# vincentjzy/OpenCorr

Hardware: AMD Instinct MI355X
Metric: converged POIs/sec (FFTCC+ICGN2D1, 33x33 subset) (higher is better)
Workload: dtype f32

## Files before the change

opencorr_amd/csrc/capi.hip:

```cpp
#include "capi_internal.h"

namespace ochip_capi {

thread_local std::string g_last_error;

int fail(int code, const char* fmt, ...) {
    char buf[512];
    va_list ap;
    va_start(ap, fmt);
    vsnprintf(buf, sizeof(buf), fmt, ap);
    va_end(ap);
    g_last_error = buf;
    return code;
}

static std::once_flag g_rocfft_once;
void rocfft_init_once() {
    std::call_once(g_rocfft_once, [] { rocfft_setup(); });
}

int create_engine(int kind, int rx, int ry, int rz, float conv, float stop, int device, oc_hip_engine** out) {
    if (!out) return fail(OC_HIP_ERR_INVALID, "null output handle");
    *out = nullptr;
    if (rx < 1 || ry < 1 || ((kind == OC_HIP_FFTCC3D || kind == OC_HIP_ICGN3D1) && rz < 1))
// ... 152 lines not shown

int run_icgn2d(oc_hip_engine* e, float* d_pois, int stride_f, size_t count, const float* d_offsets) {
    if (!e->img || e->img->ndim != 2) return fail(OC_HIP_ERR_INVALID, "ICGN2D: set_images2d has not been called");
    if (!e->ref_ready || !e->tar_ready)
        return fail(OC_HIP_ERR_INVALID, "ICGN2D: prepare() has not been called since the last set_images");
    const ImagePair& im = *e->img;
    OC_TRY(check_image2d_limits("ICGN2D", im, 1ull << 28));
    const int dof = (e->kind == OC_HIP_ICGN2D1 || e->kind == OC_HIP_ICLM2D1) ? 6 : 12;
    const bool lm = e->is_iclm();
    const bool onepass = e->arith_onepass && !lm;
    if (onepass && d_offsets)
        return fail(OC_HIP_ERR_UNSUPPORTED, "ICGN2D%d: centre offsets are not supported under arith_onepass = 1 (the one-pass kernel keeps "
                                            "integer local coordinates in a per-workgroup table); set arith_onepass = 0 for this call", dof == 6 ? 1 : 2);
    if (onepass && e->self_adaptive)
        return fail(OC_HIP_ERR_UNSUPPORTED, "ICGN2D%d: self-adaptive subset radii are not supported under arith_onepass = 1 (the one-pass "
                                            "kernel runs one radius per launch); set arith_onepass = 0", dof == 6 ? 1 : 2);
    int rx = e->rx, ry = e->ry;
    if (e->self_adaptive) {
        OC_TRY(e->cursors.reserve(2 * sizeof(int)));
        OC_HIP_TRY(ochip::launch_poi2d_max_radius(d_pois, stride_f, count, e->cursors.as<int>(), e->stream));
        int mx[2] = {0, 0};
        OC_HIP_TRY(hipMemcpyAsync(mx, e->cursors.p, sizeof(mx), hipMemcpyDeviceToHost, e->stream));
        OC_HIP_TRY(hipStreamSynchronize(e->stream));
        rx = mx[0] > 0 ? mx[0] : 1;
        ry = mx[1] > 0 ? mx[1] : 1;
        if (rx > 4096 || ry > 4096) return fail(OC_HIP_ERR_UNSUPPORTED, "ICGN2D: self-adaptive subset radius %d x %d is not plausible", rx, ry);
    }
    ochip::Icgn2dParams P = {im.ref_ptr(), e->gx.as<float>(), e->gy.as<float>(), e->coef.as<float>(),
                             im.dy,        im.dx,              rx,                ry,
                             e->conv,      e->stop,            d_offsets,         nullptr,
                             e->self_adaptive ? 1 : 0,
                             lm ? std::log((double)e->lm_lambda) : 0.0,
                             e->lm_alpha,  e->lm_beta,         e->arith_fma,      nullptr};
    const long long N = (2LL * rx + 1) * (2LL * ry + 1);
    int variant = e->icgn2d_variant;
    if (variant < 0) {
        const long long passes = ((2LL * rx + 1) * (2LL * ry + 1) + 63) / 64;
        variant = dof == 12 ? (passes <= 28 && count >= 32768 ? 4 : 3) : (passes <= 19 && count >= 32768 ? 5 : 2);
    }
    if (e->self_adaptive && (e->icgn2d_variant < 0 || ochip::icgn2d_variant_uses_table(variant))) {
        const long long passes_sa = (N + 63) / 64;
        const bool crowded = 3 * (2 * 4 * passes_sa * 256) > (160 * 1024 - 2048);
        variant = crowded ? 7 : (dof == 12 ? 3 : 2);
    }
    if (lm) variant = 1;
#if OC_BUILD_AB
    const bool band = variant == 9 && !lm && !e->self_adaptive && ochip::icgn2d_band_supported(dof, rx, ry);
#else
    const bool band = false;
#endif
    if (variant == 9 && !band) variant = dof == 12 ? 3 : 2;
    if (onepass && N > ochip::icgn2d_onepass_max_samples())
        return fail(OC_HIP_ERR_UNSUPPORTED, "ICGN2D%d: subset %dx%d (%lld samples) exceeds the one-pass kernel's on-chip limit of %d samples",
                    dof == 6 ? 1 : 2, 2 * rx + 1, 2 * ry + 1, N, ochip::icgn2d_onepass_max_samples());
    if (onepass) variant = dof == 6 ? 5 : 4;
    if (!band && !onepass && N > ochip::icgn2d_max_samples(variant)) variant = 1;
    if (!band && !onepass && N > ochip::icgn2d_max_samples(variant))
        return fail(OC_HIP_ERR_UNSUPPORTED, "ICGN2D%d: subset %dx%d (%lld samples) exceeds the on-chip limit of %d samples",
                    dof == 6 ? 1 : 2, 2 * rx + 1, 2 * ry + 1, N, ochip::icgn2d_max_samples(variant));
    if (variant == 8 && !lm) {
        OC_TRY(e->setup_recs.reserve(count * (size_t)ochip::icgn2d_setup_record_floats(dof) * sizeof(float)));
        P.setup = e->setup_recs.as<float>();
    }
    const size_t kMaxGrid = 1u << 30;
    e->setup_cache_last = 0;
    const bool cached = e->icgn2d_setup_cache && !onepass && !lm && !band && !d_offsets && !e->self_adaptive && (variant == 4 || variant == 5) &&
// ... 472 lines not shown
    for (oc_hip_engine* r : e->replicas) {
        oc_hip_engine* twin = nullptr;
        for (oc_hip_engine* d : donor->replicas)
            if (d->device == r->device && d->img && d->img->ndim == donor->img->ndim && d->img->dx == donor->img->dx &&
                d->img->dy == donor->img->dy && d->img->dz == donor->img->dz)
                twin = d;
        if (twin && r->device != e->device) {
            std::lock_guard<std::mutex> rlock(r->mu);
            r->img = twin->img;
            r->ref_ready = r->tar_ready = false;
            r->ref_generation++;
        } else {
            OC_TRY(replicate_images(e, r));
        }
    }
    return OC_HIP_OK;
}

static int clone_engine(const oc_hip_engine* e, int device, oc_hip_engine** out) {
    OC_TRY(create_engine(e->kind, e->rx, e->ry, e->rz, e->conv, e->stop, device, out));
    oc_hip_engine* r = *out;
    r->is_replica = true;
    r->lm_lambda = e->lm_lambda;
    r->lm_alpha = e->lm_alpha;
    r->lm_beta = e->lm_beta;
    r->icgn2d_tile_px = e->icgn2d_tile_px;
    r->icgn2d_variant = e->icgn2d_variant;
    r->self_adaptive = e->self_adaptive;
    r->icgn2d_xcd = e->icgn2d_xcd;
    r->arith_fma = e->arith_fma;
    r->arith_onepass = e->arith_onepass;
    r->icgn2d_split_chunks = e->icgn2d_split_chunks;
    r->icgn2d_setup_cache = e->icgn2d_setup_cache;
    r->fftcc2d_fused = e->fftcc2d_fused;
    r->fftcc3d_fused = e->fftcc3d_fused;
    r->fftcc3d_planes_blocks = e->fftcc3d_planes_blocks;
    r->icgn3d_mapping = e->icgn3d_mapping;
    r->icgn3d_tile_vox = e->icgn3d_tile_vox;
    r->fftcc3d_tile_vox = e->fftcc3d_tile_vox;
    r->host_chunk = e->host_chunk;
    r->group_allgather = e->group_allgather;
    r->group_force_rccl = e->group_force_rccl;
    return OC_HIP_OK;
}

static int rehome(oc_hip_engine* e, int device) {
    int ndev = 0;
    OC_HIP_TRY(hipGetDeviceCount(&ndev));
    if (device < 0 || device >= ndev) return fail(OC_HIP_ERR_INVALID, "device %d out of range [0,%d)", device, ndev);
    OC_HIP_TRY(hipSetDevice(e->device));
    drain_engine(e);
    e->tail_marked = false;
    clear_events(e);
    e->fft.destroy();
    e->fft.work_fwd.release();
    e->fft.work_inv.release();
    for (DevBuf* b : {&e->gx, &e->gy, &e->gz, &e->coef, &e->coef_gx, &e->coef_gy, &e->tmp, &e->poi_stage, &e->off_stage, &e->cursors,
                      &e->perm, &e->tiles, &e->perm_slots, &e->split_scratch, &e->split_tmp, &e->prefilter_tmp, &e->st_box, &e->st_counts, &e->st_start, &e->st_cursor, &e->st_slots,
                      &e->st_order, &e->st_recs, &e->st_fallback, &e->win, &e->freq, &e->norms, &e->flags, &e->group_mirror,
                      &e->group_off_mirror, &e->setup_cache_recs, &e->setup_cache_xy, &e->setup_cache_word})
        b->release();
    e->setup_cache_valid = false;
    e->setup_cache_last = 0;
    e->img.reset();
    e->ref_ready = e->tar_ready = false;
    e->st_count = 0;
    if (e->order_ev) { (void)hipEventDestroy(e->order_ev); e->order_ev = nullptr; }
    if (e->switch_ev) { (void)hipEventDestroy(e->switch_ev); e->switch_ev = nullptr; }
    if (e->group_ev) { (void)hipEventDestroy(e->group_ev); e->group_ev = nullptr; }
    for (hipEvent_t ev : e->chunk_done) (void)hipEventDestroy(ev);
    for (hipEvent_t ev : e->chunk_in) (void)hipEventDestroy(ev);
    e->chunk_done.clear();
    e->chunk_in.clear();
    if (e->copy_stream) { (void)hipStreamDestroy(e->copy_stream); e->copy_stream = nullptr; }
    if (e->copy_in_stream) { (void)hipStreamDestroy(e->copy_in_stream); e->copy_in_stream = nullptr; }
    for (hipEvent_t ev : e->split_ev) (void)hipEventDestroy(ev);
    e->split_ev.clear();
    if (e->aux_stream) { (void)hipStreamSynchronize(e->aux_stream); (void)hipStreamDestroy(e->aux_stream); e->aux_stream = nullptr; }
    (void)hipStreamDestroy(e->own_stream);
    e->own_stream = nullptr;
    OC_HIP_TRY(hipSetDevice(device));
    e->device = device;
    OC_HIP_TRY(hipStreamCreateWithFlags(&e->own_stream, hipStreamNonBlocking));
    e->stream = e->own_stream;
    return OC_HIP_OK;
}

int oc_hip_set_devices(oc_hip_engine* e, const int* device_ids, int n_devices) {
    OC_TRY(check_engine(e));
    DeviceScope device_scope;
    if (e->is_replica) return fail(OC_HIP_ERR_INVALID, "set_devices: this handle is a group member");
    if (!device_ids || n_devices < 1) return fail(OC_HIP_ERR_INVALID, "set_devices: need at least one device id");
    if (e->kind == OC_HIP_CALIBRATION || e->kind == OC_HIP_STEREOVISION)
        return fail(OC_HIP_ERR_UNSUPPORTED, "set_devices: Calibration / Stereovision handles stay on the device they were created for");
    if (n_devices > 1 && (e->kind == OC_HIP_STRAIN || e->kind == OC_HIP_REGION_FIT))
        return fail(OC_HIP_ERR_UNSUPPORTED, "set_devices: Strain / RegionFit need every neighbour of a POI and stay on one device");
    int ndev = 0;
    OC_HIP_TRY(hipGetDeviceCount(&ndev));
// ... 141 lines not shown

int oc_hip_set_tuning(oc_hip_engine* e, const char* key, int value) {
    OC_TRY(check_engine(e));
    if (!key) return fail(OC_HIP_ERR_INVALID, "null tuning key");
    std::lock_guard<std::mutex> lock(e->mu);
    const std::string k(key);
    if (k == "icgn2d_variant") {
        if (value < -1 || value >= ochip::icgn2d_variant_count())
            return fail(OC_HIP_ERR_INVALID, "icgn2d_variant %d out of range [-1 (automatic), %d)", value, ochip::icgn2d_variant_count());
        if (value >= 0 && !ochip::icgn2d_variant_built(value))
            return fail(OC_HIP_ERR_UNSUPPORTED, "icgn2d_variant %d is an A/B partner that only the A/B build of the library contains "
                                               "(python -m opencorr_amd.build --ab)", value);
        e->icgn2d_variant = value;
    } else if (k == "icgn2d_xcd" || k == "xcd") {
        e->icgn2d_xcd = value != 0;
    } else if (k == "arith_fma") {
        if (value != 0 && !(e->is_icgn2d() || e->kind == OC_HIP_ICGN3D1))
            return fail(OC_HIP_ERR_UNSUPPORTED, "arith_fma: only the ICGN2D1 / ICGN2D2 / ICLM2D1 / ICLM2D2 / ICGN3D1 engines have a fused-arithmetic build");
        e->arith_fma = value != 0;
    } else if (k == "arith_onepass") {
        if (value != 0 && !(e->kind == OC_HIP_ICGN2D1 || e->kind == OC_HIP_ICGN2D2))
            return fail(OC_HIP_ERR_UNSUPPORTED, "arith_onepass: only the ICGN2D1 / ICGN2D2 engines have a one-pass build");
        e->arith_onepass = value != 0;
    } else if (k == "icgn2d_split_chunks") {
#if !OC_BUILD_AB
        if (value != 0)
            return fail(OC_HIP_ERR_UNSUPPORTED, "icgn2d_split_chunks belongs to icgn2d_variant 8, an A/B partner that only the A/B build of the "
                                                "library contains (python -m opencorr_amd.build --ab)");
#endif
        if (value < 0 || value > 256) return fail(OC_HIP_ERR_INVALID, "icgn2d_split_chunks must be 0 (back to back) ... 256");
        e->icgn2d_split_chunks = value;
    } else if (k == "icgn2d_setup_cache") {
        e->icgn2d_setup_cache = value != 0;
    } else if (k == "icgn2d_tile_px") {
        if (value < 0 || (value > 0 && value < 16)) return fail(OC_HIP_ERR_INVALID, "icgn2d_tile_px must be 0 (off) or >= 16");
        e->icgn2d_tile_px = value;
    } else if (k == "fftcc2d_fused") {
        e->fftcc2d_fused = value == 2 ? 2 : (value != 0);
    } else if (k == "fftcc3d_fused") {
#if !OC_BUILD_AB
        if (value == 2)
            return fail(OC_HIP_ERR_UNSUPPORTED, "fftcc3d_fused = 2 (the 32^3 kernel of rounds 1 - 5) is an A/B partner that only the A/B build of the "
                                                "library contains (python -m opencorr_amd.build --ab)");
#endif
        e->fftcc3d_fused = value == 2 ? 2 : (value != 0);
    } else if (k == "fftcc3d_tile_vox") {
        if (value < 0 || (value > 0 && value < 8)) return fail(OC_HIP_ERR_INVALID, "fftcc3d_tile_vox must be 0 (off) or >= 8");
        e->fftcc3d_tile_vox = value;
    } else if (k == "icgn3d_tile_vox") {
        if (value < 0 || (value > 0 && value < 8)) return fail(OC_HIP_ERR_INVALID, "icgn3d_tile_vox must be 0 (off) or >= 8");
        e->icgn3d_tile_vox = value;
    } else if (k == "icgn3d_mapping") {
#if !OC_BUILD_AB
        if (value != 0)
            return fail(OC_HIP_ERR_UNSUPPORTED, "icgn3d_mapping = 1 (the row mapping, measured 12 - 25 %% slower) is an A/B partner that only "
                                               "the A/B build of the library contains (python -m opencorr_amd.build --ab)");
#endif
        e->icgn3d_mapping = value != 0;
    } else if (k == "fftcc3d_planes_blocks") {
        if (value < 0 || value > 4096) return fail(OC_HIP_ERR_INVALID, "fftcc3d_planes_blocks must be 0 (default) ... 4096");
        e->fftcc3d_planes_blocks = value;
    } else if (k == "single_combine") {
        e->single_combine = value != 0;
    } else if (k == "host_chunk") {
        if (value < 0 || (value > 0 && value < 16384)) return fail(OC_HIP_ERR_INVALID, "host_chunk must be 0 (off) or >= 16384 POIs");
        e->host_chunk = value;
// ... 21 lines not shown
        e->ref_ready = true;
        for (oc_hip_engine* r : e->replicas) OC_TRY(oc_hip_prepare_ref(r));
        return OC_HIP_OK;
    }
    if (im.ndim == 2) {
        OC_TRY(e->gx.reserve(bytes));
        OC_TRY(e->gy.reserve(bytes));
        OC_HIP_TRY(ochip::launch_grad2d(im.ref_ptr(), im.dy, im.dx, e->gx.as<float>(), e->gy.as<float>(), e->stream));
    } else {
        OC_TRY(e->gx.reserve(bytes));
        OC_TRY(e->gy.reserve(bytes));
        OC_TRY(e->gz.reserve(bytes));
        OC_HIP_TRY(ochip::launch_grad3d(im.ref_ptr(), im.dz, im.dy, im.dx, e->gx.as<float>(), e->gy.as<float>(),
                                        e->gz.as<float>(), e->stream));
    }
    e->ref_ready = true;
    e->ref_generation++;
    OC_TRY(mark_tail(e));
    for (oc_hip_engine* r : e->replicas) OC_TRY(oc_hip_prepare_ref(r));
    OC_HIP_TRY(hipSetDevice(e->device));
    return OC_HIP_OK;
}

int oc_hip_prepare_tar(oc_hip_engine* e) {
    OC_ACTIVATE(e);
    if (!e->is_icgn()) return OC_HIP_OK;
    if (!e->img) return fail(OC_HIP_ERR_INVALID, "prepare: set_images has not been called");
    std::lock_guard<std::mutex> lock(e->mu);
    TailGuard tail(e);
    OC_TRY(order_after_default_stream(e));
    const ImagePair& im = *e->img;
    if (im.ndim == 2) {
        OC_TRY(check_image2d_limits(e->kind == OC_HIP_NR2D1 ? "NR2D1" : "ICGN2D", im, e->kind == OC_HIP_NR2D1 ? 1ull << 26 : 1ull << 28));
        OC_TRY(e->coef.reserve(im.count() * 16 * sizeof(float)));
        OC_HIP_TRY(ochip::launch_bspline2d_lut(im.tar_ptr(), im.dy, im.dx, e->coef.as<float>(), e->stream));
        if (e->kind == OC_HIP_NR2D1) {
            OC_TRY(e->gx.reserve(im.count() * sizeof(float)));
            OC_TRY(e->gy.reserve(im.count() * sizeof(float)));
            OC_TRY(e->coef_gx.reserve(im.count() * 16 * sizeof(float)));
            OC_TRY(e->coef_gy.reserve(im.count() * 16 * sizeof(float)));
            OC_HIP_TRY(ochip::launch_grad2d(im.tar_ptr(), im.dy, im.dx, e->gx.as<float>(), e->gy.as<float>(), e->stream));
            OC_HIP_TRY(ochip::launch_bspline2d_lut(e->gx.as<float>(), im.dy, im.dx, e->coef_gx.as<float>(), e->stream));
            OC_HIP_TRY(ochip::launch_bspline2d_lut(e->gy.as<float>(), im.dy, im.dx, e->coef_gy.as<float>(), e->stream));
        }
    } else {
        OC_TRY(e->coef.reserve(im.count() * sizeof(float)));
        OC_TRY(e->prefilter_tmp.reserve(im.count() * sizeof(float)));
        OC_HIP_TRY(ochip::launch_bspline3d_prefilter(im.tar_ptr(), im.dz, im.dy, im.dx, e->coef.as<float>(),
                                                     e->prefilter_tmp.as<float>(), e->stream));
    }
    e->tar_ready = true;
    OC_TRY(mark_tail(e));
    for (oc_hip_engine* r : e->replicas) OC_TRY(oc_hip_prepare_tar(r));
    OC_HIP_TRY(hipSetDevice(e->device));
    return OC_HIP_OK;
}

int oc_hip_prepare(oc_hip_engine* e) {
    OC_TRY(oc_hip_prepare_ref(e));
    return oc_hip_prepare_tar(e);
}

}


extern "C" {

static int compute_impl(oc_hip_engine* e, void* pois, const float* offsets, size_t count, size_t stride_bytes, int memory) {
// ... 276 lines not shown
    std::lock_guard<std::mutex> lock(e->mu);
    e->self_adaptive = enable != 0;
    for (oc_hip_engine* r : e->replicas) OC_TRY(oc_hip_set_self_adaptive(r, enable));
    return OC_HIP_OK;
}

int oc_hip_synchronize(oc_hip_engine* e) {
    OC_ACTIVATE(e);
    OC_HIP_TRY(hipStreamSynchronize(e->stream));
    return OC_HIP_OK;
}

int oc_hip_get_kind(const oc_hip_engine* e, int* kind) {
    OC_TRY(check_engine(e));
    if (!kind) return fail(OC_HIP_ERR_INVALID, "null kind");
    *kind = e->kind;
    return OC_HIP_OK;
}

int oc_hip_get_field(const oc_hip_engine* e, const char* name, const float** ptr, size_t* count) {
    OC_TRY(check_engine(e));
    if (!name || !ptr || !count) return fail(OC_HIP_ERR_INVALID, "null argument");
    *ptr = nullptr;
    *count = 0;
    if (!e->img) return fail(OC_HIP_ERR_INVALID, "get_field(%s): no images set", name);
    const size_t n = e->img->count();
    const std::string s(name);
    if (s == "ref") { *ptr = e->img->ref_ptr(); *count = n; }
    else if (s == "tar") { *ptr = e->img->tar_ptr(); *count = n; }
    else if (s == "gx" && e->ref_ready) { *ptr = e->gx.as<float>(); *count = n; }
    else if (s == "gy" && e->ref_ready) { *ptr = e->gy.as<float>(); *count = n; }
    else if (s == "gz" && e->ref_ready && e->is3d()) { *ptr = e->gz.as<float>(); *count = n; }
    else if (s == "lut" && e->tar_ready && !e->is3d()) { *ptr = e->coef.as<float>(); *count = n * 16; }
    else if (s == "lut_gx" && e->tar_ready && e->kind == OC_HIP_NR2D1) { *ptr = e->coef_gx.as<float>(); *count = n * 16; }
    else if (s == "lut_gy" && e->tar_ready && e->kind == OC_HIP_NR2D1) { *ptr = e->coef_gy.as<float>(); *count = n * 16; }
    else if (s == "coef" && e->tar_ready && e->is3d()) { *ptr = e->coef.as<float>(); *count = n; }
    else return fail(OC_HIP_ERR_INVALID, "get_field: '%s' is unknown or not built yet", name);
    return OC_HIP_OK;
}

int oc_hip_read_field(oc_hip_engine* e, const char* name, float* host_dst, size_t count) {
    OC_ACTIVATE(e);
    const float* p = nullptr;
    size_t n = 0;
    OC_TRY(oc_hip_get_field(e, name, &p, &n));
    if (!host_dst || count != n) return fail(OC_HIP_ERR_INVALID, "read_field(%s): expected %zu floats, got %zu", name, n, count);
    OC_HIP_TRY(hipMemcpyAsync(host_dst, p, n * sizeof(float), hipMemcpyDeviceToHost, e->stream));
    OC_HIP_TRY(hipStreamSynchronize(e->stream));
    return OC_HIP_OK;
}

int oc_hip_profile_enable(oc_hip_engine* e, int enable) {
    OC_TRY(check_engine(e));
    std::lock_guard<std::mutex> lock(e->mu);
    e->prof = enable != 0;
    return OC_HIP_OK;
}

int oc_hip_profile_reset(oc_hip_engine* e) {
    OC_ACTIVATE(e);
    std::lock_guard<std::mutex> lock(e->mu);
    OC_HIP_TRY(hipStreamSynchronize(e->stream));
    clear_events(e);
    return OC_HIP_OK;
}

// ... 32 lines not shown
```

opencorr_amd/csrc/capi_internal.h:

```cpp
#pragma once
#include "../../include/opencorr_hip.h"

#include <hip/hip_runtime.h>
#include <rocfft/rocfft.h>

#include <dlfcn.h>

#include <algorithm>
#include <atomic>
#include <chrono>
#include <cmath>
#include <condition_variable>
#include <cstdarg>
#include <cstdio>
#include <cstdlib>
#include <cstring>
#include <memory>
#include <mutex>
#include <string>
#include <thread>
#include <vector>

#if __has_include(<rccl/rccl.h>)
#include <rccl/rccl.h>
// ... 129 lines not shown
    int rx = 0, ry = 0, rz = 0;
    float conv = 0.001f, stop = 10.f;
    hipStream_t own_stream = nullptr;
    hipStream_t stream = nullptr;
    hipEvent_t order_ev = nullptr;
    hipEvent_t switch_ev = nullptr;
    bool tail_marked = false;
    std::shared_ptr<ImagePair> img;
    DevBuf gx, gy, gz, coef;
    DevBuf coef_gx, coef_gy;
    DevBuf tmp;
    DevBuf prefilter_tmp;
    bool ref_ready = false, tar_ready = false;
    DevBuf poi_stage, off_stage;
    DevBuf cursors;
    DevBuf perm, tiles, perm_slots;
    DevBuf setup_recs;
    DevBuf setup_cache_recs, setup_cache_xy, setup_cache_word;
    struct SetupCacheKey {
        size_t count = 0;
        int stride_f = 0, variant = -1, dof = 0, rx = 0, ry = 0, arith_fma = 0, height = 0, width = 0;
        const void *ref = nullptr, *gx = nullptr, *gy = nullptr;
        unsigned long long ref_generation = 0;
        bool operator==(const SetupCacheKey& o) const {
            return count == o.count && stride_f == o.stride_f && variant == o.variant && dof == o.dof && rx == o.rx && ry == o.ry &&
                   arith_fma == o.arith_fma && height == o.height && width == o.width && ref == o.ref && gx == o.gx && gy == o.gy &&
                   ref_generation == o.ref_generation;
        }
    } setup_cache_key;
    bool setup_cache_valid = false;
    unsigned long long ref_generation = 0;
    unsigned setup_cache_epoch = 0;
    int setup_cache_last = 0;
    int icgn2d_setup_cache = 1;
    DevBuf split_scratch, split_tmp;
    float st_radius = 0.f, st_zncc = 0.9f;
    int st_nmin = 0, st_approx = 1, st_ndim = 0;
    size_t st_count = 0;
    ochip::StrainGrid st_grid{};
    DevBuf st_box, st_counts, st_start, st_cursor, st_slots, st_order, st_recs, st_fallback;
    float cal_i[13] = {}, cal_e[6] = {};
    float cal_K[9] = {}, cal_R[9] = {}, cal_T[3] = {}, cal_P[12] = {};
    float cal_conv = 0.001f;
    int cal_iter = 40, cal_h = 0, cal_w = 0;
    DevBuf cal_map_x, cal_map_y, cal_stage;
    oc_hip_engine* stereo_cam[2] = {nullptr, nullptr};
    float stereo_F[9] = {};
    float lm_lambda = 100.f, lm_alpha = 0.1f, lm_beta = 10.f;
    int icgn2d_tile_px = 128;
    FftPlans fft;
    DevBuf win, freq, norms, flags;
    int icgn2d_variant = -1;
    bool self_adaptive = false;
    int icgn2d_xcd = 1;
    int arith_fma = 0;
    int arith_onepass = 0;
    int fftcc2d_fused = 1;
    int fftcc3d_fused = 1;
    int fftcc3d_planes_blocks = 0;
    int fftcc3d_tile_vox = 64;
    int icgn3d_tile_vox = 64;
    int icgn3d_mapping = 0;
    hipStream_t copy_stream = nullptr, copy_in_stream = nullptr;
    hipStream_t aux_stream = nullptr;
    std::vector<hipEvent_t> split_ev;
    int icgn2d_split_chunks = 0;
// ... 159 lines not shown
```

opencorr_amd/csrc/icgn2d.hip:

```cpp
#include <atomic>
#include <cstdlib>
#include <type_traits>

#include "dic2d_device.h"
#include "oc_kernels.h"
#ifndef OC_ABLATE2D
#define OC_ABLATE2D 0
#endif
#ifndef OC_SWEEP_BARRIER
#define OC_SWEEP_BARRIER -1
#endif
#ifndef OC_SWEEP_PRIO
#define OC_SWEEP_PRIO 0
#endif
#ifndef OC_SETUP_BATCH
#define OC_SETUP_BATCH 6
#endif
#ifndef OC_HESS_BATCH
#define OC_HESS_BATCH 6
#endif
#ifndef OC_NUM_BATCH
#define OC_NUM_BATCH 6
#endif
#ifndef OC_V5_G
// ... 116 lines not shown
    int rx = P.rx, ry = P.ry;
    if (P.self_adaptive) {
        rx = (int)wave_bcast(rec, poi2d::SRX);
        ry = (int)wave_bcast(rec, poi2d::SRY);
        if (rx < 0 || ry < 0 || (2 * rx + 1) * (2 * ry + 1) > NTA * kWave) {
            if (lane == 0) poi[poi2d::ZNCC] = zncc_in >= 0 ? -3.f : zncc_in;
            leave();
            return;
        }
    }
    float offx = 0.f, offy = 0.f;
    if constexpr (OFFS) {
        offx = uni(P.offsets[2 * idx]);
        offy = uni(P.offsets[2 * idx + 1]);
    }

    const bool guard_geo = py - ry < 0 || px - rx < 0 || py + ry > height - 1 || px + rx > width - 1;
    const bool guard_data = fabsf(u_in) >= width || fabsf(v_in) >= height || zncc_in < 0 || isnan(u_in) || isnan(v_in);
    if (guard_geo || (guard_data && !cache_fill)) {
        if (lane == 0) poi[poi2d::ZNCC] = zncc_in >= 0 ? -3.f : zncc_in;
        leave();
        return;
    }
    const int W = 2 * rx + 1, N = W * (2 * ry + 1);
    const float fN = (float)N;
    const int NT = (N + kWave - 1) / kWave;
    const int NF = N / kWave;
    const int q64 = kWave / W, r64 = kWave - q64 * W;
    const int r0 = lane / W;
    const int c0 = lane - r0 * W;
    const unsigned goff = (unsigned)__builtin_amdgcn_readfirstlane((((int)py - ry) * width + ((int)px - rx)) * 4);
    const __amdgpu_buffer_rsrc_t r_gx = make_rsrc(P.gx), r_gy = make_rsrc(P.gy), r_ref = make_rsrc(P.ref);
    const LutPlanes4 r_lut(P.lut, height, width);
    const unsigned w4 = (unsigned)width * 4u;
    auto soff = [&](const SampleWalk& w) { return __umul24((unsigned)w.r, w4) + ((unsigned)w.c << 2); };

    auto tab_at = [&](int t) { return tab_xy[t * kWave + lane]; };
    auto off_at = [&](int t) { return tab_off[t * kWave + lane]; };

    float ref_norm, ref_mean;
    const int x0r = (int)(px - rx), y0r = (int)(py - ry);
    const unsigned roff = (unsigned)__builtin_amdgcn_readfirstlane((y0r * width + x0r) * 4);
    float* const setup_rec = (kSetupOnly || kIterOnly) ? P.setup + idx * (unsigned long long)kSetupFloats
                             : (CACHE && (cache_fill || cache_use)) ? P.cache_recs + idx * (unsigned long long)kSetupFloats
                                                                     : nullptr;
    if (kIterOnly || cache_use) {
        ref_mean = uni(setup_rec[0]);
        ref_norm = uni(setup_rec[1]);
    } else if constexpr (kSetupOnly) {
        float acc = 0.f;
        passes_batched<kSetupBatch>(
            NF, NT, (NF * kWave + lane) < N,
            [&](int t, bool valid) { return valid ? buf_f32(r_ref, off_at(t), roff) : 0.f; },
            [&](int, bool valid, float v) { acc = valid ? acc + v : acc; });
        const float mean = wave_allreduce_sum(acc) / fN;
        ref_mean = uni(mean);
        acc = 0.f;
        passes_batched<kSetupBatch>(
            NF, NT, (NF * kWave + lane) < N,
            [&](int t, bool valid) { return valid ? buf_f32(r_ref, off_at(t), roff) : 0.f; },
            [&](int, bool valid, float v) {
                const float d = v - mean;
                acc = valid ? mad(d, d, acc) : acc;
            });
        ref_norm = uni(sqrtf(wave_allreduce_sum(acc)));
    } else {
// ... 238 lines not shown
    for (int i = 0; i < 12; i++) cur[i] = 0.f;
    float znssd0 = 4.f, lambda = 0.f;
    if constexpr (LM) {
        cur[0] = u_in; cur[1] = ux_in; cur[2] = uy_in;
        cur[6] = v_in; cur[7] = vx_in; cur[8] = vy_in;
    }
#if OC_ABLATE2D & 4
    LutFetch f_stale[G] = {};
#endif
#pragma nounroll
    do {
        iter++;
        if constexpr (DOF == 12) {
#pragma unroll
            for (int k = 0; k < 6; k++) {
                row3[k] = wave_bcast(Wcol[3], k);
                row4[k] = wave_bcast(Wcol[4], k);
            }
        }
        lap(3);
        bool negative = false;
        float acc = 0.f;
        constexpr bool kCornerTest = DOF == 6 && LM == 0 && !(OC_ABLATE2D & 6);
        if constexpr (kCornerTest) {
            const float cxl = (float)((lane & 1) ? rx : -rx) - offx, cyl = (float)((lane & 2) ? ry : -ry) - offy;
            const float cax = tcx + (mad(Wm[1], cyl, Wm[0] * cxl) + Wm[2]), cay = tcy + (mad(Wm[4], cyl, Wm[3] * cxl) + Wm[5]);
            const int cxi = floor_to_int(cax), cyi = floor_to_int(cay);
            const bool cout = (unsigned)(cxi - 1) > (unsigned)(width - 4) || (unsigned)(cyi - 1) > (unsigned)(height - 4);
            if (!(OC_ABLATE2D & 1) && wave_any(cout)) {
                if (lane == 0) poi[poi2d::ZNCC] = -3.f;
                return;
            }
        }
        {
            SampleWalk w(lane, r0, c0, W, q64, r64);
            constexpr bool kWarpV = (OC_UNIFORM_IN_VGPR & 1) != 0 && DOF == 6, kSizeV = (OC_UNIFORM_IN_VGPR & 2) != 0;
            float Wv[6];
#pragma unroll
            for (int i = 0; i < 6; i++) Wv[i] = kWarpV ? in_vgpr(Wm[i]) : Wm[i];
            const float tcxv = kWarpV ? in_vgpr(tcx) : tcx, tcyv = kWarpV ? in_vgpr(tcy) : tcy;
            const int heightv = kSizeV ? in_vgpr(height) : height, widthv = kSizeV ? in_vgpr(width) : width;
            auto issue = [&](LutFetch(&f)[G], bool(&valid)[G], int t0, auto checked) {
                constexpr bool CHECKED = decltype(checked)::value;
#pragma unroll
                for (int g = 0; g < G; g++, w.next()) {
                    valid[g] = CHECKED ? w.s < N : true;
                    float xl, yl;
                    if constexpr (TAB) {
                        const f2 lxy = tab_at(CHECKED ? min(t0 + g, NT - 1) : t0 + g);
                        xl = lxy.x - offx;
                        yl = lxy.y - offy;
                    } else {
                        xl = (float)(w.c - rx) - offx;
                        yl = (float)(w.r - ry) - offy;
                    }
                    float wx, wy;
                    if constexpr (DOF == 6) {
                        wx = mad(Wv[1], yl, Wv[0] * xl) + Wv[2];
                        wy = mad(Wv[4], yl, Wv[3] * xl) + Wv[5];
                    } else {
                        const float pv[6] = {xl * xl, xl * yl, yl * yl, xl, yl, 1.f};
                        wx = row3[0] * pv[0];
                        wy = row4[0] * pv[0];
#pragma unroll
                        for (int k = 1; k < 6; k++) {
                            wx = mad(row3[k], pv[k], wx);
// ... 11 lines not shown
                        f[g].dx = __builtin_amdgcn_fractf(ax);
                        f[g].dy = __builtin_amdgcn_fractf(ay);
                        r_lut.load(f[g], (__umul24((unsigned)yi, (unsigned)widthv) + (unsigned)xi) << 4);
                    } else if constexpr ((OC_ABLATE2D & 6) != 0) {
                        unsigned off = lut_locate<LM != 0>(f[g], heightv, widthv, ax, ay, out);
                        if (OC_ABLATE2D & 2) off = iter > 1 ? (off & 0x3ff0u) : off;
                        if (!(OC_ABLATE2D & 4) || iter == 1) r_lut.load(f[g], off);
                    } else {
                        lut_fetch<LM != 0>(f[g], r_lut, heightv, widthv, ax, ay, out);
                    }
                    if constexpr (!LM && !kCornerTest) negative = negative || out;
                }
            };
            auto consume = [&](const LutFetch(&f)[G], const bool(&valid)[G], int t0, auto checked) {
                constexpr bool CHECKED = decltype(checked)::value;
#pragma unroll
                for (int g = 0; g < G; g++) {
#if OC_ABLATE2D & 8
                    const float v = iter > 1 ? f[g].c0.x + f[g].c1.y * f[g].dx + f[g].c2.z * f[g].dy + f[g].c3.w : lut_value(f[g]);
#else
                    const float v = LM ? lut_eval(f[g]) : lut_value(f[g]);
#endif
                    if constexpr (CHECKED) {
                        negative = negative || (valid[g] && v < 0.f);
                        acc = valid[g] ? acc + v : acc;
                        if (t0 + g < NT) l_ts[(t0 + g) * kWave] = v;
                    } else {
                        negative = negative || v < 0.f;
                        acc = acc + v;
                        l_ts[(t0 + g) * kWave] = v;
                    }
                }
            };
            const int full_groups = NF / G;
            int t0 = 0;
#pragma nounroll
            for (int q = 0; q < full_groups; q++, t0 += G) {
                if constexpr (SWEEP_SYNC > 0) {
                    if (q % SWEEP_SYNC == 0) __builtin_amdgcn_s_barrier();
                }
#if OC_ABLATE2D & 4
                LutFetch(&f)[G] = f_stale;
#else
                LutFetch f[G];
#endif
                bool valid[G];
#if OC_SWEEP_PRIO == 1
                __builtin_amdgcn_s_setprio(2);
#elif OC_SWEEP_PRIO == 2
                __builtin_amdgcn_s_setprio(0);
#endif
                issue(f, valid, t0, std::false_type{});
#if OC_SWEEP_PRIO == 1
                __builtin_amdgcn_s_setprio(0);
#elif OC_SWEEP_PRIO == 2
                __builtin_amdgcn_s_setprio(2);
#endif
                consume(f, valid, t0, std::false_type{});
            }
#if OC_SWEEP_PRIO
            __builtin_amdgcn_s_setprio(0);
#endif
#pragma nounroll
            for (; t0 < NT; t0 += G) {
#if OC_ABLATE2D & 4
                LutFetch(&f)[G] = f_stale;
#else
                LutFetch f[G];
#endif
                bool valid[G];
                issue(f, valid, t0, std::true_type{});
                consume(f, valid, t0, std::true_type{});
            }
        }
        lap(2);
        if constexpr (!LM) {
            if (!(OC_ABLATE2D & 1) && wave_any(negative)) {
                if (lane == 0) poi[poi2d::ZNCC] = -3.f;
                return;
            }
        }
        float tmean = wave_allreduce_sum(acc) / fN;
        if constexpr ((OC_UNIFORM_IN_VGPR & 4) != 0) tmean = in_vgpr(tmean);
        acc = 0.f;
#pragma unroll 6
        for (int t = 0; t < NF; t++) {
            const float d = l_ts[t * kWave] - tmean;
            acc = mad(d, d, acc);
        }
        if (NF < NT) {
            const float d = l_ts[NF * kWave] - tmean;
            acc = (NF * kWave + lane) < N ? mad(d, d, acc) : acc;
        }
        const float tar_norm = uni(sqrtf(wave_allreduce_sum(acc)));
        float factor = ref_norm / tar_norm;
        float ref_mean_v = ref_mean;
        if constexpr ((OC_UNIFORM_IN_VGPR & 4) != 0) {
// ... 415 lines not shown
```

opencorr_amd/csrc/oc_kernels.h:

```cpp
#pragma once

#include <hip/hip_runtime.h>
#include <stddef.h>

#ifndef OC_BUILD_AB
#define OC_BUILD_AB 0
#endif

namespace ochip {

hipError_t launch_grad2d(const float* img, int height, int width, float* gx, float* gy, hipStream_t stream);
hipError_t launch_bspline2d_lut(const float* img, int height, int width, float* lut, hipStream_t stream);
hipError_t launch_colmajor_to_rowmajor(const float* src, int height, int width, float* dst, hipStream_t stream);

struct Icgn2dParams {
    const float* ref;
    const float* gx;
    const float* gy;
    const float* lut;
    int height, width;
    int rx, ry;
    float conv, stop;
    const float* offsets;
    const unsigned* perm;
    int self_adaptive;
    double lm_log_lambda;
    float lm_alpha, lm_beta;
    int arith_fma;
    float* setup;
    float* cache_recs;
    const unsigned* cache_word;
    unsigned cache_epoch;
    int cache_force_fill;
};
hipError_t launch_poi2d_max_radius(const float* pois, int stride_floats, size_t count, int* out2, hipStream_t stream);
hipError_t launch_icgn2d1(const Icgn2dParams& p, float* pois, int stride_floats, size_t count, int variant, bool xcd,
                          hipStream_t stream, int phase = 0);
hipError_t launch_iclm2d1(const Icgn2dParams& p, float* pois, int stride_floats, size_t count, bool xcd, hipStream_t stream);
hipError_t launch_iclm2d2(const Icgn2dParams& p, float* pois, int stride_floats, size_t count, bool xcd, hipStream_t stream);
int iclm2d_max_samples();
hipError_t launch_icgn2d2(const Icgn2dParams& p, float* pois, int stride_floats, size_t count, int variant, bool xcd,
                          hipStream_t stream, int phase = 0);
int icgn2d_setup_record_floats(int dof);
#define OC_DECLARE_ICGN2D_LAUNCHERS                                                                                          \
    hipError_t launch_icgn2d1(const Icgn2dParams& p, float* pois, int stride_floats, size_t count, int variant, bool xcd,   \
                              hipStream_t stream, int phase);                                                               \
    hipError_t launch_icgn2d2(const Icgn2dParams& p, float* pois, int stride_floats, size_t count, int variant, bool xcd,   \
                              hipStream_t stream, int phase);                                                               \
    hipError_t launch_iclm2d1(const Icgn2dParams& p, float* pois, int stride_floats, size_t count, bool xcd, hipStream_t stream); \
    hipError_t launch_iclm2d2(const Icgn2dParams& p, float* pois, int stride_floats, size_t count, bool xcd, hipStream_t stream);
namespace sep {
OC_DECLARE_ICGN2D_LAUNCHERS
}
namespace fma {
OC_DECLARE_ICGN2D_LAUNCHERS
}
#undef OC_DECLARE_ICGN2D_LAUNCHERS
hipError_t launch_icgn2d1_band(const Icgn2dParams& p, float* pois, int stride_floats, size_t count, bool xcd, hipStream_t stream);
hipError_t launch_icgn2d2_band(const Icgn2dParams& p, float* pois, int stride_floats, size_t count, bool xcd, hipStream_t stream);
bool icgn2d_band_supported(int dof, int rx, int ry);
namespace sep {
hipError_t launch_icgn2d1_band(const Icgn2dParams& p, float* pois, int stride_floats, size_t count, bool xcd, hipStream_t stream);
hipError_t launch_icgn2d2_band(const Icgn2dParams& p, float* pois, int stride_floats, size_t count, bool xcd, hipStream_t stream);
}
namespace fma {
hipError_t launch_icgn2d1_band(const Icgn2dParams& p, float* pois, int stride_floats, size_t count, bool xcd, hipStream_t stream);
// ... 195 lines not shown
```

opencorr_amd/csrc/prepare2d.hip:

```cpp
#include "oc_device.h"
#include "oc_kernels.h"

namespace ochip {

__global__ __launch_bounds__(256) void grad2d_kernel(const float* __restrict__ img, int height, int width,
                                                     float* __restrict__ gx, float* __restrict__ gy) {
    const float first_factor = 1.f / 12.f;
    const float second_factor = 2.f / 3.f;
    const int c = blockIdx.x * blockDim.x + threadIdx.x;
    const int r = blockIdx.y;
    if (c >= width) return;
    const size_t g = (size_t)r * width + c;
    float vx = 0.f, vy = 0.f;
    if (c >= 2 && c < width - 2) {
        float result = 0.0f;
        result -= img[g + 2] * first_factor;
        result += img[g + 1] * second_factor;
        result -= img[g - 1] * second_factor;
        result += img[g - 2] * first_factor;
        vx = result;
    }
    if (r >= 2 && r < height - 2) {
        float result = 0.0f;
        result -= img[g + 2 * (size_t)width] * first_factor;
        result += img[g + (size_t)width] * second_factor;
        result -= img[g - (size_t)width] * second_factor;
        result += img[g - 2 * (size_t)width] * first_factor;
        vy = result;
    }
    gx[g] = vx;
    gy[g] = vy;
}

__device__ constexpr float kBC[4][4] = {
    {-144.0f / 336.0f, 384.0f / 336.0f, -384.0f / 336.0f, 144.0f / 336.0f},
    {342.0f / 336.0f, -702.0f / 336.0f, 450.0f / 336.0f, -90.0f / 336.0f},
    {-198.0f / 336.0f, -18.0f / 336.0f, 270.0f / 336.0f, -54.0f / 336.0f},
    {0.0f, 1.0f, 0.0f, 0.0f}};

__global__ __launch_bounds__(256) void bspline2d_lut_kernel(const float* __restrict__ img, int height, int width,
                                                            float* __restrict__ lut) {
    const int c = blockIdx.x * blockDim.x + threadIdx.x;
    const int r = blockIdx.y;
    if (c >= width) return;
    const size_t plane = (size_t)height * width;
    float4* out = reinterpret_cast<float4*>(lut) + ((size_t)r * width + c);
    if (r < 1 || r >= height - 2 || c < 1 || c >= width - 2) {
        const float4 z = make_float4(0.f, 0.f, 0.f, 0.f);
        out[0] = z; out[plane] = z; out[2 * plane] = z; out[3 * plane] = z;
        return;
    }
    float q[4][4];
#pragma unroll
    for (int i = 0; i < 4; i++)
#pragma unroll
        for (int j = 0; j < 4; j++) q[i][j] = img[(size_t)(r - 1 + i) * width + (c - 1 + j)];
    float pm[4][4];
#pragma unroll
    for (int k = 0; k < 4; k++)
#pragma unroll
        for (int l = 0; l < 4; l++) {
            float acc = 0.f;
#pragma unroll
            for (int m = 0; m < 4; m++)
#pragma unroll
                for (int n = 0; n < 4; n++) acc += kBC[l][m] * kBC[k][n] * q[n][m];
            pm[k][l] = acc;
        }
#pragma unroll
    for (int k = 0; k < 4; k++) out[k * plane] = make_float4(pm[3 - k][3], pm[3 - k][2], pm[3 - k][1], pm[3 - k][0]);
}

__global__ __launch_bounds__(256) void colmajor_to_rowmajor_kernel(const float* __restrict__ src, int height,
                                                                   int width, float* __restrict__ dst) {
    __shared__ float tile[32][33];
    const int tx = threadIdx.x & 31, ty = threadIdx.x >> 5;
    const int r0 = blockIdx.y * 32, c0 = blockIdx.x * 32;
    for (int j = ty; j < 32; j += 8) {
        int c = c0 + j, r = r0 + tx;
        if (c < width && r < height) tile[j][tx] = src[(size_t)c * height + r];
    }
    __syncthreads();
    for (int j = ty; j < 32; j += 8) {
        int r = r0 + j, c = c0 + tx;
        if (r < height && c < width) dst[(size_t)r * width + c] = tile[tx][j];
    }
}

constexpr int kGradRows = 16;
__global__ __launch_bounds__(256) void grad2d4_kernel(const float* __restrict__ img, int height, int width,
                                                      float* __restrict__ gx, float* __restrict__ gy) {
    const float first_factor = 1.f / 12.f;
    const float second_factor = 2.f / 3.f;
    const int c = (blockIdx.x * blockDim.x + threadIdx.x) * 4;
    const int r0 = blockIdx.y * kGradRows;
    if (c >= width) return;
    const int r1 = min(r0 + kGradRows, height);
    auto row4 = [&](int r) -> float4 {
        if (r < 0 || r >= height) return make_float4(0.f, 0.f, 0.f, 0.f);
        return *reinterpret_cast<const float4*>(img + (size_t)r * width + c);
    };
    float4 m2 = row4(r0 - 2), m1 = row4(r0 - 1), c0 = row4(r0), p1 = row4(r0 + 1);
    auto comp = [&](float a2, float a1, float b1, float b2) {
// ... 11 lines not shown
        const float2 lo = *reinterpret_cast<const float2*>(img + g - (c >= 4 ? 2 : 0));
        const float2 hi = *reinterpret_cast<const float2*>(img + g + (c + 8 <= width ? 4 : 0));
        const float f[8] = {lo.x, lo.y, c0.x, c0.y, c0.z, c0.w, hi.x, hi.y};
        float vx[4], vy[4];
#pragma unroll
        for (int t = 0; t < 4; t++) {
            const int cc = c + t;
            vx[t] = (cc >= 2 && cc < width - 2) ? comp(f[t + 4], f[t + 3], f[t + 1], f[t]) : 0.f;
        }
        const bool ry = r >= 2 && r < height - 2;
        vy[0] = ry ? comp(p2.x, p1.x, m1.x, m2.x) : 0.f;
        vy[1] = ry ? comp(p2.y, p1.y, m1.y, m2.y) : 0.f;
        vy[2] = ry ? comp(p2.z, p1.z, m1.z, m2.z) : 0.f;
        vy[3] = ry ? comp(p2.w, p1.w, m1.w, m2.w) : 0.f;
        *reinterpret_cast<float4*>(gx + g) = make_float4(vx[0], vx[1], vx[2], vx[3]);
        *reinterpret_cast<float4*>(gy + g) = make_float4(vy[0], vy[1], vy[2], vy[3]);
        m2 = m1; m1 = c0; c0 = p1; p1 = p2;
    }
}

hipError_t launch_grad2d(const float* img, int height, int width, float* gx, float* gy, hipStream_t stream) {
    (void)hipGetLastError();
    const bool vec = (width & 3) == 0 && ((reinterpret_cast<uintptr_t>(img) | reinterpret_cast<uintptr_t>(gx) | reinterpret_cast<uintptr_t>(gy)) & 15) == 0;
    if (vec) {
        dim3 block(256), grid((width / 4 + 255) / 256, (height + kGradRows - 1) / kGradRows);
        hipLaunchKernelGGL(grad2d4_kernel, grid, block, 0, stream, img, height, width, gx, gy);
    } else {
        dim3 block(256), grid((width + 255) / 256, height);
        hipLaunchKernelGGL(grad2d_kernel, grid, block, 0, stream, img, height, width, gx, gy);
    }
    return hipGetLastError();
}

hipError_t launch_bspline2d_lut(const float* img, int height, int width, float* lut, hipStream_t stream) {
    dim3 block(256), grid((width + 255) / 256, height);
    (void)hipGetLastError();
    hipLaunchKernelGGL(bspline2d_lut_kernel, grid, block, 0, stream, img, height, width, lut);
    return hipGetLastError();
}

hipError_t launch_colmajor_to_rowmajor(const float* src, int height, int width, float* dst, hipStream_t stream) {
    dim3 block(256), grid((width + 31) / 32, (height + 31) / 32);
    (void)hipGetLastError();
    hipLaunchKernelGGL(colmajor_to_rowmajor_kernel, grid, block, 0, stream, src, height, width, dst);
    return hipGetLastError();
}

}
```

Measured before the change: 73.77 million.

## Add integer-displacement fast path sampling precomputed B-spline value plane in ICGN2D

The B-spline LUT kernel now also writes a value plane holding the interpolated intensity at integer positions. In the ICGN2D sweep, when the warp is pure integer translation (unit deformation, integral shift and POI coordinates, subset fully inside), each sample reads one float from that plane instead of fetching four float4 LUT coefficients and evaluating the bicubic. This targets the first iteration after FFTCC, where the initial guess is an integer shift. It costs an extra plane of memory and a write during LUT setup, plus a uniform branch and added code in the inner loop.

```diff
diff --git a/opencorr_amd/csrc/capi.hip b/opencorr_amd/csrc/capi.hip
--- a/opencorr_amd/csrc/capi.hip
+++ b/opencorr_amd/csrc/capi.hip
@@ -208,6 +208,7 @@
                              e->self_adaptive ? 1 : 0,
                              lm ? std::log((double)e->lm_lambda) : 0.0,
                              e->lm_alpha,  e->lm_beta,         e->arith_fma,      nullptr};
+    P.lut_val = (e->icgn2d_int_first && e->tar_ready && e->coef_has_val) ? e->coef.as<float>() + im.count() * 16 : nullptr;
     const long long N = (2LL * rx + 1) * (2LL * ry + 1);
     int variant = e->icgn2d_variant;
     if (variant < 0) {
@@ -746,6 +747,7 @@
     r->arith_onepass = e->arith_onepass;
     r->icgn2d_split_chunks = e->icgn2d_split_chunks;
     r->icgn2d_setup_cache = e->icgn2d_setup_cache;
+    r->icgn2d_int_first = e->icgn2d_int_first;
     r->fftcc2d_fused = e->fftcc2d_fused;
     r->fftcc3d_fused = e->fftcc3d_fused;
     r->fftcc3d_planes_blocks = e->fftcc3d_planes_blocks;
@@ -778,6 +780,7 @@
     e->setup_cache_last = 0;
     e->img.reset();
     e->ref_ready = e->tar_ready = false;
+    e->coef_has_val = false;
     e->st_count = 0;
     if (e->order_ev) { (void)hipEventDestroy(e->order_ev); e->order_ev = nullptr; }
     if (e->switch_ev) { (void)hipEventDestroy(e->switch_ev); e->switch_ev = nullptr; }
@@ -985,6 +988,8 @@
         e->icgn2d_split_chunks = value;
     } else if (k == "icgn2d_setup_cache") {
         e->icgn2d_setup_cache = value != 0;
+    } else if (k == "icgn2d_int_first") {
+        e->icgn2d_int_first = value != 0;
     } else if (k == "icgn2d_tile_px") {
         if (value < 0 || (value > 0 && value < 16)) return fail(OC_HIP_ERR_INVALID, "icgn2d_tile_px must be 0 (off) or >= 16");
         e->icgn2d_tile_px = value;
@@ -1072,8 +1077,12 @@
     const ImagePair& im = *e->img;
     if (im.ndim == 2) {
         OC_TRY(check_image2d_limits(e->kind == OC_HIP_NR2D1 ? "NR2D1" : "ICGN2D", im, e->kind == OC_HIP_NR2D1 ? 1ull << 26 : 1ull << 28));
-        OC_TRY(e->coef.reserve(im.count() * 16 * sizeof(float)));
-        OC_HIP_TRY(ochip::launch_bspline2d_lut(im.tar_ptr(), im.dy, im.dx, e->coef.as<float>(), e->stream));
+        const bool with_val = e->kind == OC_HIP_ICGN2D1 || e->kind == OC_HIP_ICGN2D2;
+        e->coef_has_val = false;
+        OC_TRY(e->coef.reserve(im.count() * (with_val ? 17 : 16) * sizeof(float)));
+        OC_HIP_TRY(ochip::launch_bspline2d_lut(im.tar_ptr(), im.dy, im.dx, e->coef.as<float>(), e->stream,
+                                               with_val ? e->coef.as<float>() + im.count() * 16 : nullptr));
+        e->coef_has_val = with_val;
         if (e->kind == OC_HIP_NR2D1) {
             OC_TRY(e->gx.reserve(im.count() * sizeof(float)));
             OC_TRY(e->gy.reserve(im.count() * sizeof(float)));
@@ -1416,6 +1425,7 @@
     else if (s == "gy" && e->ref_ready) { *ptr = e->gy.as<float>(); *count = n; }
     else if (s == "gz" && e->ref_ready && e->is3d()) { *ptr = e->gz.as<float>(); *count = n; }
     else if (s == "lut" && e->tar_ready && !e->is3d()) { *ptr = e->coef.as<float>(); *count = n * 16; }
+    else if (s == "lut_val" && e->tar_ready && !e->is3d() && e->coef_has_val) { *ptr = e->coef.as<float>() + n * 16; *count = n; }
     else if (s == "lut_gx" && e->tar_ready && e->kind == OC_HIP_NR2D1) { *ptr = e->coef_gx.as<float>(); *count = n * 16; }
     else if (s == "lut_gy" && e->tar_ready && e->kind == OC_HIP_NR2D1) { *ptr = e->coef_gy.as<float>(); *count = n * 16; }
     else if (s == "coef" && e->tar_ready && e->is3d()) { *ptr = e->coef.as<float>(); *count = n; }
diff --git a/opencorr_amd/csrc/capi_internal.h b/opencorr_amd/csrc/capi_internal.h
--- a/opencorr_amd/csrc/capi_internal.h
+++ b/opencorr_amd/csrc/capi_internal.h
@@ -185,6 +185,8 @@
     unsigned long long ref_generation = 0;
     unsigned setup_cache_epoch = 0;
     int setup_cache_last = 0;
+    int icgn2d_int_first = 1;
+    bool coef_has_val = false;
     int icgn2d_setup_cache = 1;
     DevBuf split_scratch, split_tmp;
     float st_radius = 0.f, st_zncc = 0.9f;
diff --git a/opencorr_amd/csrc/icgn2d.hip b/opencorr_amd/csrc/icgn2d.hip
--- a/opencorr_amd/csrc/icgn2d.hip
+++ b/opencorr_amd/csrc/icgn2d.hip
@@ -172,6 +172,8 @@
     const unsigned goff = (unsigned)__builtin_amdgcn_readfirstlane((((int)py - ry) * width + ((int)px - rx)) * 4);
     const __amdgpu_buffer_rsrc_t r_gx = make_rsrc(P.gx), r_gy = make_rsrc(P.gy), r_ref = make_rsrc(P.ref);
     const LutPlanes4 r_lut(P.lut, height, width);
+    constexpr bool kIntSweep = LM == 0 && OFFS == 0 && PHASE != 1 && OC_ABLATE2D == 0;
+    const __amdgpu_buffer_rsrc_t r_val = make_rsrc(kIntSweep && P.lut_val ? P.lut_val : P.lut);
     const unsigned w4 = (unsigned)width * 4u;
     auto soff = [&](const SampleWalk& w) { return __umul24((unsigned)w.r, w4) + ((unsigned)w.c << 2); };
 
@@ -476,6 +478,31 @@
                 return;
             }
         }
+        bool int_sweep = false;
+        unsigned val_base = 0;
+        if constexpr (kIntSweep) {
+            if (P.lut_val != nullptr && !P.self_adaptive) {
+                float tu, tv;
+                bool unit;
+                if constexpr (DOF == 6) {
+                    tu = Wm[2];
+                    tv = Wm[5];
+                    unit = Wm[0] == 1.f && Wm[1] == 0.f && Wm[3] == 0.f && Wm[4] == 1.f;
+                } else {
+                    tu = row3[5];
+                    tv = row4[5];
+                    unit = row3[0] == 0.f && row3[1] == 0.f && row3[2] == 0.f && row3[3] == 1.f && row3[4] == 0.f &&
+                           row4[0] == 0.f && row4[1] == 0.f && row4[2] == 0.f && row4[3] == 0.f && row4[4] == 1.f;
+                }
+                constexpr float kExact = 4194304.f;
+                const bool integral = truncf(tu) == tu && truncf(tv) == tv && truncf(px) == px && truncf(py) == py &&
+                                      fabsf(tu) < kExact && fabsf(tv) < kExact && fabsf(px) < kExact && fabsf(py) < kExact;
+                const int x0 = integral ? (int)px + (int)tu - rx : 0, y0 = integral ? (int)py + (int)tv - ry : 0;
+                const bool inside = x0 >= 1 && y0 >= 1 && x0 + 2 * rx <= width - 3 && y0 + 2 * ry <= height - 3;
+                int_sweep = __builtin_amdgcn_readfirstlane((int)(unit && integral && inside)) != 0;
+                val_base = (unsigned)__builtin_amdgcn_readfirstlane(int_sweep ? (y0 * width + x0) * 4 : 0);
+            }
+        }
         {
             SampleWalk w(lane, r0, c0, W, q64, r64);
             constexpr bool kWarpV = (OC_UNIFORM_IN_VGPR & 1) != 0 && DOF == 6, kSizeV = (OC_UNIFORM_IN_VGPR & 2) != 0;
@@ -553,6 +580,32 @@
                     }
                 }
             };
+            auto short_group = [&](int t0, auto checked) {
+                constexpr bool CHECKED = decltype(checked)::value;
+                float v[G];
+                bool valid[G];
+#pragma unroll
+                for (int g = 0; g < G; g++, w.next()) {
+                    valid[g] = CHECKED ? w.s < N : true;
+                    unsigned off;
+                    if constexpr (TAB) off = off_at(CHECKED ? min(t0 + g, NT - 1) : t0 + g);
+                    else off = soff(w);
+                    if constexpr (CHECKED) off = valid[g] ? off : 0u;
+                    v[g] = buf_f32(r_val, off, val_base);
+                }
+#pragma unroll
+                for (int g = 0; g < G; g++) {
+                    if constexpr (CHECKED) {
+                        negative = negative || (valid[g] && v[g] < 0.f);
+                        acc = valid[g] ? acc + v[g] : acc;
+                        if (t0 + g < NT) l_ts[(t0 + g) * kWave] = v[g];
+                    } else {
+                        negative = negative || v[g] < 0.f;
+                        acc = acc + v[g];
+                        l_ts[(t0 + g) * kWave] = v[g];
+                    }
+                }
+            };
             const int full_groups = NF / G;
             int t0 = 0;
 #pragma nounroll
@@ -560,6 +613,12 @@
                 if constexpr (SWEEP_SYNC > 0) {
                     if (q % SWEEP_SYNC == 0) __builtin_amdgcn_s_barrier();
                 }
+                if constexpr (kIntSweep) {
+                    if (int_sweep) {
+                        short_group(t0, std::false_type{});
+                        continue;
+                    }
+                }
 #if OC_ABLATE2D & 4
                 LutFetch(&f)[G] = f_stale;
 #else
@@ -584,6 +643,12 @@
 #endif
 #pragma nounroll
             for (; t0 < NT; t0 += G) {
+                if constexpr (kIntSweep) {
+                    if (int_sweep) {
+                        short_group(t0, std::true_type{});
+                        continue;
+                    }
+                }
 #if OC_ABLATE2D & 4
                 LutFetch(&f)[G] = f_stale;
 #else
diff --git a/opencorr_amd/csrc/oc_kernels.h b/opencorr_amd/csrc/oc_kernels.h
--- a/opencorr_amd/csrc/oc_kernels.h
+++ b/opencorr_amd/csrc/oc_kernels.h
@@ -10,7 +10,7 @@
 namespace ochip {
 
 hipError_t launch_grad2d(const float* img, int height, int width, float* gx, float* gy, hipStream_t stream);
-hipError_t launch_bspline2d_lut(const float* img, int height, int width, float* lut, hipStream_t stream);
+hipError_t launch_bspline2d_lut(const float* img, int height, int width, float* lut, hipStream_t stream, float* value_plane = nullptr);
 hipError_t launch_colmajor_to_rowmajor(const float* src, int height, int width, float* dst, hipStream_t stream);
 
 struct Icgn2dParams {
@@ -32,6 +32,7 @@
     const unsigned* cache_word;
     unsigned cache_epoch;
     int cache_force_fill;
+    const float* lut_val;
 };
 hipError_t launch_poi2d_max_radius(const float* pois, int stride_floats, size_t count, int* out2, hipStream_t stream);
 hipError_t launch_icgn2d1(const Icgn2dParams& p, float* pois, int stride_floats, size_t count, int variant, bool xcd,
diff --git a/opencorr_amd/csrc/prepare2d.hip b/opencorr_amd/csrc/prepare2d.hip
--- a/opencorr_amd/csrc/prepare2d.hip
+++ b/opencorr_amd/csrc/prepare2d.hip
@@ -1,4 +1,4 @@
-#include "oc_device.h"
+#include "dic2d_device.h"
 #include "oc_kernels.h"
 
 namespace ochip {
@@ -39,7 +39,7 @@
     {0.0f, 1.0f, 0.0f, 0.0f}};
 
 __global__ __launch_bounds__(256) void bspline2d_lut_kernel(const float* __restrict__ img, int height, int width,
-                                                            float* __restrict__ lut) {
+                                                            float* __restrict__ lut, float* __restrict__ val) {
     const int c = blockIdx.x * blockDim.x + threadIdx.x;
     const int r = blockIdx.y;
     if (c >= width) return;
@@ -48,6 +48,7 @@
     if (r < 1 || r >= height - 2 || c < 1 || c >= width - 2) {
         const float4 z = make_float4(0.f, 0.f, 0.f, 0.f);
         out[0] = z; out[plane] = z; out[2 * plane] = z; out[3 * plane] = z;
+        if (val) val[(size_t)r * width + c] = 0.f;
         return;
     }
     float q[4][4];
@@ -69,6 +70,16 @@
         }
 #pragma unroll
     for (int k = 0; k < 4; k++) out[k * plane] = make_float4(pm[3 - k][3], pm[3 - k][2], pm[3 - k][1], pm[3 - k][0]);
+    if (val) {
+        LutFetch f;
+        f.c0 = make_float4(pm[3][3], pm[3][2], pm[3][1], pm[3][0]);
+        f.c1 = make_float4(pm[2][3], pm[2][2], pm[2][1], pm[2][0]);
+        f.c2 = make_float4(pm[1][3], pm[1][2], pm[1][1], pm[1][0]);
+        f.c3 = make_float4(pm[0][3], pm[0][2], pm[0][1], pm[0][0]);
+        f.dx = in_vgpr(0.f);
+        f.dy = in_vgpr(0.f);
+        val[(size_t)r * width + c] = lut_value(f);
+    }
 }
 
 __global__ __launch_bounds__(256) void colmajor_to_rowmajor_kernel(const float* __restrict__ src, int height,
@@ -146,10 +157,10 @@
     return hipGetLastError();
 }
 
-hipError_t launch_bspline2d_lut(const float* img, int height, int width, float* lut, hipStream_t stream) {
+hipError_t launch_bspline2d_lut(const float* img, int height, int width, float* lut, hipStream_t stream, float* value_plane) {
     dim3 block(256), grid((width + 255) / 256, height);
     (void)hipGetLastError();
-    hipLaunchKernelGGL(bspline2d_lut_kernel, grid, block, 0, stream, img, height, width, lut);
+    hipLaunchKernelGGL(bspline2d_lut_kernel, grid, block, 0, stream, img, height, width, lut, value_plane);
     return hipGetLastError();
 }
 
```

Result: faster. 82.04 million (median of 6 runs) (+11.2%).
